# YukeWang96/GNNAdvisor_OSDI21

Measured on AMD Instinct MI355X. Metric: aggregated edges/sec, GCN sum-aggregation SpMM (SAG) hidden=64, higher is better.
Workload: dtype f32; 1 GPU; reddit-like power-law graph, random node order; num_nodes=232965, nnz=114623790, dim=64, partSize=128, num_parts=1008217, parallelism=single GPU, call=GNNA.SAG (pybind module, reference signature, fresh output), decider=auto/mi355x, column_phases=16, build_id=0.6.1+877bf822ee5a343e

## Files before the change

### gnnadvisor_osdi21_amd/build.py

```python
from __future__ import annotations

import os
import subprocess
import sys
import sysconfig

PKG = os.path.dirname(os.path.abspath(__file__))
ROOT = os.path.dirname(PKG)
CSRC = os.path.join(PKG, "csrc")
INCLUDE = os.path.join(ROOT, "include")
LIB = os.path.join(CSRC, "libgnna.so")
EXT = os.path.join(PKG, "GNNAdvisor.so")
ARCH = "gfx950"
HIPCC = os.environ.get("HIPCC", "/opt/rocm/bin/hipcc")

LIB_SOURCES = [os.path.join(CSRC, f) for f in ("gnna_agg.hip", "gnna_stream.hip", "gnna_sweep.hip", "gnna_dense.hip", "gnna_x16.hip", "gnna_reduce.hip", "gnna_stats.hip", "gnna_softagg.hip", "gnna_pool.hip", "gnna_segnorm.hip", "gnna_attnpool.hip", "gnna_topk.hip", "gnna_sddmm.hip", "gnna_edge.hip", "gnna_gat.hip", "gnna_gatv2.hip", "gnna_dotattn.hip", "gnna_typed.hip", "gnna_transpose.hip", "gnna_sample.hip", "gnna_walk.hip", "gnna_edgefeat.hip", "gnna_spatial.hip",
                                                "gnna_gemm.hip", "gnna_runtime.hip", "gnna_host.cpp", "gnna_reorder.cpp")]
PUBLIC_HEADERS = ("gnna.h", "gnna_ext.h", "gnna_gatv2.h", "gnna_dotattn.h", "gnna_gat_edge.h", "gnna_stats.h", "gnna_softagg.h",
                  "gnna_pool.h", "gnna_attnpool.h", "gnna_topk.h", "gnna_segnorm.h", "gnna_walk.h", "gnna_edgefeat.h",
                  "gnna_spatial.h")
INTERNAL_HEADERS = ("gnna_internal.h", "gnna_device.h", "gnna_launch.h", "gnna_gat_common.h", "gnna_keys.h", "gnna_segments.h",
                    "gnna_parts.h")
_PUBLIC = [os.path.join(INCLUDE, f) for f in PUBLIC_HEADERS]
LIB_DEPS = LIB_SOURCES + [os.path.join(CSRC, f) for f in INTERNAL_HEADERS] + _PUBLIC
EXT_SOURCES = [os.path.join(CSRC, "gnna_torch.cpp")]
EXT_DEPS = EXT_SOURCES + _PUBLIC


def source_hash() -> str:
    import hashlib
    h = hashlib.sha256()
    for path in sorted(set(LIB_DEPS + EXT_DEPS)):
        h.update(os.path.relpath(path, ROOT).encode() + b"\0")
        with open(path, "rb") as f:
            h.update(f.read())
        h.update(b"\0")
    return h.hexdigest()[:16]
# ... 83 lines not shown
```

### gnnadvisor_osdi21_amd/csrc/gnna_agg.hip

```cpp
#include <hip/hip_runtime.h>

#include <algorithm>
#include <cmath>
#include <cstdint>
#include <cstdio>

#include "gnna.h"
#include "gnna_device.h"
#include "gnna_internal.h"

namespace gnna {
namespace {


__global__ void __launch_bounds__(kBlock)
prologue_kernel(float *__restrict__ Y, size_t n_floats, int D, int ldy, const int32_t *__restrict__ p2n,
                const int32_t *__restrict__ pp, int64_t P, int32_t *flag, int32_t seq, int validate, int zero_fill,
                const int32_t *__restrict__ chk_ids, int64_t chk_n, const unsigned long long *__restrict__ chk_sum,
                int32_t *stale_flag, uint32_t *__restrict__ clear_words, int n_clear)
{
    if (blockIdx.x == 0 && (int)threadIdx.x < n_clear) clear_words[threadIdx.x] = 0u;
    const unsigned fill_blocks = chk_ids ? gridDim.x - 1 : gridDim.x;
    if (blockIdx.x >= fill_blocks) {
        if (threadIdx.x < kWave) {
            const unsigned long long then = chk_sum[0], distrusted = chk_sum[4];
            const unsigned long long now = graph_checksum(chk_ids, chk_n, pp, P, (int)threadIdx.x);
            if (threadIdx.x == 0 && (now != then || distrusted != 0ull)) *stale_flag = seq;
        }
        return;
    }
    const size_t tid = (size_t)blockIdx.x * blockDim.x + threadIdx.x;
    const size_t nthreads = (size_t)fill_blocks * blockDim.x;
    typedef float f32x4 __attribute__((ext_vector_type(4)));
    if (!zero_fill) {
    } else if (ldy != D) {
        if ((D & 3) == 0 && (ldy & 3) == 0 && (reinterpret_cast<uintptr_t>(Y) & 15) == 0) {
            const size_t n4 = n_floats >> 2;
            const unsigned d4 = (unsigned)D >> 2, ld4 = (unsigned)ldy >> 2;
            const f32x4 z = (f32x4)(0.f);
            for (size_t i = tid; i < n4; i += nthreads) {
                const size_t r = i / d4;
                reinterpret_cast<f32x4 *>(Y)[r * ld4 + (i - r * d4)] = z;
            }
        } else {
            for (size_t i = tid; i < n_floats; i += nthreads) {
                const size_t r = i / (unsigned)D;
                Y[r * (size_t)ldy + (i - r * (unsigned)D)] = 0.f;
            }
        }
    } else if ((reinterpret_cast<uintptr_t>(Y) & 15) == 0) {
        const size_t n4 = n_floats >> 2;
        f32x4 *Y4 = reinterpret_cast<f32x4 *>(Y);
        const f32x4 z = (f32x4)(0.f);
        for (size_t i = tid; i < n4; i += nthreads) Y4[i] = z;
        for (size_t i = (n4 << 2) + tid; i < n_floats; i += nthreads) Y[i] = 0.f;
    } else {
        for (size_t i = tid; i < n_floats; i += nthreads) Y[i] = 0.f;
    }
    if (validate) {
        bool bad = false;
        for (int64_t g = (int64_t)tid; g < P; g += (int64_t)nthreads) {
            if (pp[g + 1] < pp[g]) bad = true;
            if (g + 1 < P && p2n[g + 1] < p2n[g]) bad = true;
        }
        if (bad) *flag = seq;
    }
}

__global__ void __launch_bounds__(kBlock)
sparse_prologue_kernel(float *__restrict__ Y, int64_t N, int D, int ldy, const int32_t *__restrict__ p2n,
                       const int32_t *__restrict__ pp, int64_t P, int G, int32_t *flag, int32_t seq, int validate,
                       unsigned long long *gaps, int64_t big_rows)
{
    const int lane = threadIdx.x & (kWave - 1);
    const int64_t wave = ((int64_t)blockIdx.x * blockDim.x + threadIdx.x) >> 6;
    const int64_t nwaves = ((int64_t)gridDim.x * blockDim.x) >> 6;
    typedef float f32x4 __attribute__((ext_vector_type(4)));
    const bool vec_ok = (D & 3) == 0 && (reinterpret_cast<uintptr_t>(Y) & 15) == 0;
    auto clear_rows = [&](int64_t lo, int64_t cnt) {
        if (gaps && cnt >= big_rows) {
            unsigned long long idx = 0;
// ... 75 lines not shown
        return;
    }
    if (!gaps) return;
    const unsigned long long n = gaps[0] < (unsigned long long)kGapEntries ? gaps[0] : (unsigned long long)kGapEntries;
    for (unsigned long long k = 0; k < n; k++) {
        float *base = Y + (size_t)gaps[2 + 2 * k] * (size_t)ldy;
        const size_t cnt = (size_t)gaps[3 + 2 * k] * (size_t)D;
        for (size_t i = tid; i < cnt; i += nthreads) *at(base, i) = 0.f;
    }
}

__global__ void __launch_bounds__(kBlock)
scale_rows_kernel(const float *__restrict__ X, int64_t ld_in, const float *__restrict__ deg, float *__restrict__ Xs,
                  int64_t rows, int D, int ld_out)
{
    const size_t tid = (size_t)blockIdx.x * blockDim.x + threadIdx.x;
    const size_t nthreads = (size_t)gridDim.x * blockDim.x;
    typedef float f32x4 __attribute__((ext_vector_type(4)));
    const bool aligned = ((reinterpret_cast<uintptr_t>(X) | reinterpret_cast<uintptr_t>(Xs)) & 15) == 0;
    if (ld_out == D && ld_in == D && (D & 3) == 0 && aligned) {
        const size_t n4 = ((size_t)rows * (size_t)D) >> 2;
        const int d4 = D >> 2;
        for (size_t i = tid; i < n4; i += nthreads) {
            const f32x4 v = __builtin_nontemporal_load(reinterpret_cast<const f32x4 *>(X) + i);
            reinterpret_cast<f32x4 *>(Xs)[i] = deg ? v * deg[i / d4] : v;
        }
    } else if ((D & 3) == 0 && (ld_out & 3) == 0 && (ld_in & 3) == 0 && aligned) {
        const size_t n4 = ((size_t)rows * (size_t)D) >> 2;
        const unsigned d4 = (unsigned)D >> 2;
        const size_t ldo4 = (size_t)ld_out >> 2, ldi4 = (size_t)ld_in >> 2;
        for (size_t i = tid; i < n4; i += nthreads) {
            const size_t r = i / d4, c4 = i - r * d4;
            const f32x4 v = __builtin_nontemporal_load(reinterpret_cast<const f32x4 *>(X) + r * ldi4 + c4);
            reinterpret_cast<f32x4 *>(Xs)[r * ldo4 + c4] = deg ? v * deg[r] : v;
        }
    } else {
        const size_t total = (size_t)rows * (size_t)D;
        for (size_t i = tid; i < total; i += nthreads) {
            const size_t r = i / (unsigned)D, cc = i - r * (unsigned)D;
            const float v = __builtin_nontemporal_load(X + r * (size_t)ld_in + cc);
            Xs[r * (size_t)ld_out + cc] = deg ? v * deg[r] : v;
        }
    }
}


static size_t gather_footprint_bytes(int64_t num_in_rows, int ldx, int dim)
{
    return (size_t)num_in_rows * (size_t)std::min(ldx, (std::max(dim, 4) * 4 + 127) / 128 * 32) * sizeof(float);
}

thread_local int t_last_phases = 1;
thread_local int t_last_launches = 1;

double avg_lines_per_row(int64_t row_bytes, int64_t stride_bytes)
{
    int64_t lines = 0;
    for (int k = 0; k < 32; k++) {
// ... 81 lines not shown
    const double edges = st.edges;
    if (t.sweep != 0 || deterministic || B < 2) return 0;
    if (dim <= 32 || dim > 64 || !sweep_supports(mode, dim, x_bytes)) return 0;
    if (num_in_rows != num_out_rows || x_bytes > ((size_t)160 << 20)) return 0;
    if (edges < 300.0 * (double)std::max<int64_t>(1, num_out_rows)) return 0;
    const double cap = (double)sweep_acc_rows(dim, 1) * 0.9 * (double)std::max(8, num_cus);
    if ((double)num_out_rows > 2.0 * cap) return 0;
    if (near_share(st, (double)num_in_rows / 16.0) > 0.30) return 0;
    if (t.column_phases >= 2) return B;
    return std::max(2, std::min(std::min(16, 2 * B), std::max(2, part_size / 4)));
}

constexpr double kDenseEdgeSeconds = 9.9e-12;
constexpr double kDenseChunkSeconds = 0.73e-6;
constexpr double kDenseTallChunkSeconds = 0.76e-6;
constexpr double kDenseSplitSeconds = 11.0e-6;
constexpr double kDenseLaunchSeconds = 7.0e-6;
constexpr double kDenseMinSaving = 25.0e-6;
constexpr double kDenseMinShare = 0.03;

int trimmed_hubs(int H, int num_cus)
{
    const int round = kDenseTileRanks * std::max(1, num_cus);
    return (H > round && H % round != 0 && H % round < round / 4) ? H / round * round : H;
}

double dense_block_saving(double hubs, double entries, int num_cus)
{
    if (hubs <= 0.0) return 0.0;
    const double He = (double)trimmed_hubs((int)hubs, num_cus);
    const double Hp = std::ceil(He / kDenseChunkRanks) * kDenseChunkRanks;
// ... 72 lines not shown
    const size_t n = rows * (size_t)D;
    for (size_t i = (size_t)blockIdx.x * blockDim.x + threadIdx.x; i < n; i += (size_t)gridDim.x * blockDim.x) {
        const size_t r = i / (unsigned)D, c = i - r * (unsigned)D;
        if (Y[r * ld + c] < 0.f) Y[r * ld + c] = 0.f;
    }
}
}

void launch_relu_rows(DeviceState *ds, hipStream_t stream, float *out, int64_t rows, int dim, int64_t ld)
{
    hipLaunchKernelGGL(relu_rows_kernel, dim3(elementwise_grid(rows * dim, ds->num_cus, 8)), dim3(kBlock), 0, stream, out,
                       (size_t)ld, (size_t)rows, dim);
}

namespace {

int launch_agg(int mode, const float *input, int64_t ld_in, int64_t num_in_rows, const int32_t *column_index,
               const float *degrees, const float *degrees_in, float epsilon, const int32_t *part_pointers,
               const int32_t *part2Node, float *out, int64_t ld_out, int64_t num_nodes, int dim, int64_t num_parts,
               int partSize, int dimWorker, int warpPerBlock, void *stream_v, unsigned flags,
               int num_windows = 1, int win_begin = 0, int win_end = 1, bool profiled = true, int hint_dim = 0);

int column_blocks(const gnna_tuning &tune, int dim, int64_t num_in_rows, int64_t est_edges)
{
    if (tune.wide_blocks == 2 || dim < 72) return 1;
    if (tune.wide_blocks == 1) return (dim + 63) / 64;
    const bool hot = est_edges >= 32 * num_in_rows;
    if (!hot || (size_t)num_in_rows * (size_t)dim * sizeof(float) > ((size_t)250000000)) return 1;
    const bool long_rows = est_edges >= 200 * num_in_rows;
    if (dim < (long_rows ? 100 : 192)) return 1;
// ... 78 lines not shown
        const int nb = column_blocks(tune, dim, num_in_rows, est);
        if (nb > 1)
            return launch_agg_blocked(nb, mode, input, ld_in, num_in_rows, column_index, degrees, degrees_in, epsilon, part_pointers,
                                      part2Node, out, ld_out, num_nodes, dim, num_parts, partSize, dimWorker, warpPerBlock, stream_v, flags);
    }
    int32_t *flag = nullptr;
    const int32_t seq = next_call_seq(ds, stream, &flag);
    const int prof_call = profiled ? profile_acquire_call(num_parts > 0) : -1;
    profile_record(prof_call, 0, stream);
    const int ldy = (int)ld_out;

    const size_t n_floats = (size_t)num_nodes * (size_t)dim;
    const unsigned long long *chk_sum = nullptr;
    int64_t chk_n = 0;
    int32_t *stale_flag = flag + kFlagSlots;
    auto run_prologue = [&](int sparse_G, uint32_t *clear_words = nullptr, int n_clear = 0) -> int {
        const int validate = (num_parts > 0 && !tune.trust_canonical) ? 1 : 0;
        const int zero_fill = (accumulate_into_out || win_begin > 0) ? 0 : 1;
        if (sparse_G > 0 && zero_fill && num_parts > 0) {
            int64_t blocks = (num_parts + kBlock - 1) / kBlock;
            blocks = std::max<int64_t>(1, std::min<int64_t>(blocks, (int64_t)ds->num_cus * 8));
            unsigned long long *gaps = ds->gap_lists + (size_t)call_block_of(ds, stream, seq) * kGapWords;
            (void)hipMemsetAsync(gaps, 0, sizeof(unsigned long long), stream);
            const int64_t big_rows = std::max<int64_t>(64, ((int64_t)1 << 20) / std::max(1, dim * 4));
            hipLaunchKernelGGL(sparse_prologue_kernel, dim3((unsigned)blocks), dim3(kBlock), 0, stream, out, num_nodes, dim, ldy,
                               part2Node, part_pointers, num_parts, sparse_G, flag, seq, validate, gaps, big_rows);
            hipLaunchKernelGGL(post_prologue_kernel, dim3((unsigned)(ds->num_cus * 8)), dim3(kBlock), 0, stream, out,
                               n_floats, dim, ldy, flag, seq, gaps);
        } else {
            size_t work = std::max(n_floats / 4, (size_t)num_parts);
            int64_t blocks = (int64_t)((work + kBlock - 1) / kBlock);
            blocks = std::max<int64_t>(1, std::min<int64_t>(blocks, (int64_t)ds->num_cus * 8));
            hipLaunchKernelGGL(prologue_kernel, dim3((unsigned)blocks + (chk_sum ? 1u : 0u)), dim3(kBlock), 0, stream, out, n_floats,
                               dim, ldy, part2Node, part_pointers, num_parts, flag, seq, validate, zero_fill,
// ... 29 lines not shown
            direct = aligned16 && avg_lines_per_row((int64_t)dim * 4, ld_in * 4) <= avg_lines_per_row((int64_t)dim * 4, (int64_t)want * 4) + 1e-9;
    }
    const int ldx = direct ? (int)ld_in : want;
    const float *X = input;
    const float *row_scale = nullptr;
    float eps = epsilon;
    const size_t x_bytes = (size_t)num_in_rows * (size_t)ldx * sizeof(float);
    const size_t foot_bytes = gather_footprint_bytes(num_in_rows, ldx, dim);
    const bool wide = x_bytes > 0xffffffffull;
    if (!direct) {
        void *xs = nullptr;
        rc = get_workspace(ds, stream, 1, x_bytes, &xs);
        if (rc != GNNA_OK) return rc;
        const int64_t r0 = std::min<int64_t>((int64_t)win_begin * window_rows, num_in_rows);
        const int64_t r1 = std::min<int64_t>((int64_t)win_end * window_rows, num_in_rows);
        const size_t s_bytes = (size_t)(r1 - r0) * (size_t)dim * sizeof(float);
        int64_t sblocks = (int64_t)((s_bytes / 16 + kBlock - 1) / kBlock);
        sblocks = std::max<int64_t>(1, std::min<int64_t>(sblocks, (int64_t)ds->num_cus * 8));
        hipLaunchKernelGGL(scale_rows_kernel, dim3((unsigned)sblocks), dim3(kBlock), 0, stream,
                           input + (size_t)r0 * (size_t)ld_in, ld_in, prescale ? degrees_in + r0 : nullptr,
                           static_cast<float *>(xs) + (size_t)r0 * ldx, r1 - r0, dim, ldx);
        hipError_t es = hipGetLastError();
        if (es != hipSuccess) return fail(GNNA_ERR_HIP, "staging launch: %s", hipGetErrorString(es));
        X = static_cast<const float *>(xs);
        if (prescale) {
            row_scale = degrees;
            eps = 1.f;
            mode = MODE_GIN;
        }
    }

    int B = 1;
    const uint8_t *cnt = nullptr;
    int S = kMaxSlices;
    int win_lo = 0, win_hi = 0;
    SlicePlan plan;
    const bool can_slice = num_parts >= 1024 && num_in_rows >= 64 && foot_bytes >= ((size_t)2 << 20);
    if (windowed) {
// ... 42 lines not shown
                                tune.ids_check_every);
            if (rc != GNNA_OK) return rc;
            if (sw_ids) count_event(CTR_PACKED_LAUNCHES);
        }
        DenseBlock db;
        const int32_t *res_ids = nullptr; const uint32_t *res_off = nullptr;
        bool dense = false;
        if (sw_ids && plan.pinned && !relu && dim >= kDenseMinDim && dim <= kDenseMaxDim && num_in_rows == num_nodes && tune.column_phases < 2 &&
            plan_dense_block(plan.handle, &db) && !db.off && db.res_plan && db.res_cnt && (auto_Bs > 0 || db.forced)) {
            rc = get_packed_ids(ds, stream, db.res_plan, Bs, kWave, false, false, &res_ids, &res_off);
            if (rc != GNNA_OK) return rc;
            dense = true;
        }
        uint32_t *sync = ds->sweep_sync + (size_t)call_block_of(ds, stream, seq) * kSweepSlotWords;
        static_assert(kXcds * 16 + 2 <= kBlock, "the prologue clears the sweep counters with one block");
        rc = run_prologue(0, sync, kXcds * 16 + 2);
        if (rc != GNNA_OK) return rc;
        SweepLaunch w;
        w.mode = mode; w.X = X; w.col = column_index; w.pp = part_pointers; w.p2n = part2Node; w.Y = out;
        w.cnt = cnt; w.row_scale = row_scale; w.flag = flag; w.seq = seq; w.trust = tune.trust_canonical ? 1 : 0; w.sync = sync;
        w.P = num_parts; w.D = dim; w.ldx = ldx; w.ldy = ldy; w.S = S; w.B = Bs;
        w.relu = relu; w.num_out_rows = num_nodes;
        w.U = std::max(tune.loads_in_flight, 8);
        w.rows_with_edges = plan.stats.valid ? (int64_t)std::min((double)num_nodes, plan.stats.groups) : num_nodes;
        if (tune.groups_per_chunk > 64) w.rounds = tune.groups_per_chunk / 64;
        w.slack = tune.sweep_slack; w.wgs_per_cu = tune.blocks_per_cu;
        w.dynamic = tune.xcd_remap != 0;
        w.plain_ok = !accumulate_into_out; w.eps = eps;
        w.ids_packed = sw_ids; w.item_off = sw_off; w.packed_stale = stale_flag;
        if (dense) { w.res_col = db.res_col; w.res_pp = db.res_pp; w.res_cnt = db.res_cnt; w.res_ids_packed = res_ids; w.res_item_off = res_off; }
        t_last_phases = Bs;
        t_last_launches = 1;
        void *hub_image = nullptr;
        if (dense) {
            rc = get_workspace(ds, stream, kSlotDenseImage, dense_image_bytes(db.H_pad), &hub_image);
            if (rc != GNNA_OK) return rc;
            rc = launch_hub_split(stream, db, X, ldx, dim, hub_image, stale_flag, seq);
            if (rc != GNNA_OK) return rc;
        }
        rc = launch_sweep(ds, w, stream);
        if (rc != GNNA_OK) return rc;
        if (dense) {
            rc = launch_hub_block(ds, stream, db, hub_image, out, ldy, dim, mode == MODE_GIN, eps, row_scale, stale_flag, seq);
            if (rc != GNNA_OK) return rc;
        }
        profile_record(prof_call, 2, stream);
        return GNNA_OK;
    }

    int G = std::min(64, tune.groups_per_chunk * B);
    if (mode == MODE_EDGE && cnt && !windowed && plan.handle && plan.pinned && (plan.stats.valid || tune.sweep == 1) &&
// ... 377 lines not shown
```

### gnnadvisor_osdi21_amd/csrc/gnna_dense.hip

```cpp
#include <hip/hip_runtime.h>

#include <algorithm>
#include <cmath>
#include <cstdint>
#include <cstdio>
#include <cstdlib>
#include <vector>

#include "gnna.h"
#include "gnna_device.h"
#include "gnna_internal.h"

namespace gnna {
namespace {

constexpr int kHubBuckets = 64;
constexpr int kHubMax = 16384;
constexpr int kHubThreads = 512;
constexpr int kHubWaves = kHubThreads / kWave;
constexpr int kHubTileM = kDenseTileRanks;
constexpr int kHubKC = kDenseChunkRanks;
static_assert(kHubTileM == 32, "a tile row of the bitmap per 32 destination ranks");
constexpr int kSplitThreads = 128;
static_assert(kHubKC % (2 * kHubTileM) == 0 && (kHubTileM * 64) % kHubThreads == 0, "whole tiles per chunk, elements per thread");
static_assert(kDenseMaxDim <= 64, "the split image holds 64 columns");

__host__ __device__ inline int hub_bucket(int64_t d)
{
    if (d <= 1) return 0;
    int k = 0;
    while ((d >> (k + 1)) != 0) k++;
    const int b = 2 * k + ((d * d >= ((int64_t)1 << (2 * k + 1))) ? 1 : 0);
    return b < kHubBuckets ? b : kHubBuckets - 1;
}

__global__ void __launch_bounds__(kBlock)
hub_degree_kernel(const int32_t *__restrict__ pp, const int32_t *__restrict__ p2n, int64_t P, int64_t N, int32_t *__restrict__ deg)
{
// ... 134 lines not shown
    int32_t seq;
    int H_pad, D, ldy;
    int scaled;
    float eps;
};

struct SplitParams {
    const float *X;
    const int32_t *r2n;
    unsigned char *img;
    const int32_t *stale;
    int32_t seq;
    int D, ldx;
};

typedef typename VecOf<4>::T HubVT;
typedef int HubIT __attribute__((ext_vector_type(4)));

constexpr int kHubFrag = 1024;
constexpr int kHubPiece = 16 * kHubFrag;
constexpr int kHubImage = 3 * kHubPiece;
static_assert(kHubKC == 128 && kHubTileM == 32 && kHubWaves == 8, "the shape hub_block_kernel is written for");

typedef __bf16 HubFrag __attribute__((ext_vector_type(8)));
typedef uint32_t HubU4 __attribute__((ext_vector_type(4)));
typedef uint32_t HubU2 __attribute__((ext_vector_type(2)));

__device__ __forceinline__ void hub_split(uint32_t x, uint32_t &hi, uint32_t &mid, uint32_t &lo)
{
    hi = x & 0xffff0000u;
    const float r = __uint_as_float(x) - __uint_as_float(hi);
    mid = __float_as_uint(r) & 0xffff0000u;
    lo = __float_as_uint(r - __uint_as_float(mid));
}

__device__ __forceinline__ uint32_t hub_pack(uint32_t first, uint32_t second) { return __builtin_amdgcn_perm(second, first, 0x07060302u); }

__device__ __forceinline__ HubFrag hub_ones(uint32_t bits)
{
    const uint32_t y = bits | (bits << 15);
    HubU4 v;
#pragma unroll
    for (int i = 0; i < 4; i++) v[i] = ((y >> (2 * i)) & 0x10001u) * 0x3f80u;
    return __builtin_bit_cast(HubFrag, v);
}

template <bool FULL>
__global__ void __launch_bounds__(kSplitThreads)
hub_split_kernel(const SplitParams p)
{
    if (*p.stale == p.seq) return;
    __shared__ __attribute__((aligned(16))) unsigned char s_img[3 * 4 * kHubFrag];
    const int t = (int)threadIdx.x;
    const int g = t >> 4, pc = t & 15;
    const int step = (int)blockIdx.x;
    const int D = p.D;
    const HubIT node = *reinterpret_cast<const HubIT *>(&p.r2n[step * 32 + 4 * g]);
    HubVT v[4];
#pragma unroll
    for (int k = 0; k < 4; k++) {
        const int nd = node[k];
        const float *src = p.X + (size_t)(nd < 0 ? 0 : nd) * (size_t)p.ldx + 4 * pc;
        HubVT x = (HubVT)(0.f);
        if (nd >= 0) {
            if constexpr (FULL) {
                if (4 * pc < D) x = *reinterpret_cast<const HubVT *>(src);
            } else {
#pragma unroll
                for (int q = 0; q < 4; q++)
                    if (4 * pc + q < D) x[q] = src[q];
            }
        }
        v[k] = x;
    }
    const int wbase = (pc >> 2) * kHubFrag + (16 * (g >> 1) + 4 * (pc & 3)) * 16 + 8 * (g & 1);
#pragma unroll
    for (int cc = 0; cc < 4; cc++) {
        uint32_t pk[3][2];
#pragma unroll
        for (int h = 0; h < 2; h++) {
            uint32_t a[3], b[3];
            hub_split(__float_as_uint(v[2 * h][cc]), a[0], a[1], a[2]);
            hub_split(__float_as_uint(v[2 * h + 1][cc]), b[0], b[1], b[2]);
#pragma unroll
            for (int i = 0; i < 3; i++) pk[i][h] = hub_pack(a[i], b[i]);
        }
#pragma unroll
        for (int i = 0; i < 3; i++) {
            HubU2 o;
            o[0] = pk[i][0];
            o[1] = pk[i][1];
            *reinterpret_cast<HubU2 *>(&s_img[wbase + i * 4 * kHubFrag + cc * 16]) = o;
        }
    }
    __syncthreads();
    unsigned char *out = p.img + (size_t)(step >> 2) * kHubImage + (size_t)(step & 3) * 4 * kHubFrag;
#pragma unroll
    for (int u = 0; u < 3 * 4 * kHubFrag / 16 / kSplitThreads; u++) {
        const int idx = u * kSplitThreads + t;
        const int i = idx >> 8, off = (idx & 255) * 16;
        *reinterpret_cast<HubU4 *>(&out[i * kHubPiece + off]) = *reinterpret_cast<const HubU4 *>(&s_img[i * 4 * kHubFrag + off]);
    }
}

template <int NT, int TM>
__global__ void __launch_bounds__(kHubThreads)
hub_block_kernel(const HubParams p)
{
    if (*p.stale == p.seq) return;
    constexpr int TR = TM / 32;
    static_assert((TM == kHubTileM || TM == 2 * kHubTileM) && (NT == 3 || NT == 4), "tile shapes");
    __shared__ __attribute__((aligned(16))) float s_part[4 * TM * 64];
    const int tid = (int)threadIdx.x;
    const int lane = tid & (kWave - 1);
    const int wib = __builtin_amdgcn_readfirstlane(tid >> 6);
    const int chunks = p.H_pad / kHubKC;
    const int steps = p.H_pad >> 5;
// ... 294 lines not shown
```

### gnnadvisor_osdi21_amd/csrc/gnna_launch.h

```cpp
#ifndef GNNA_LAUNCH_H_
#define GNNA_LAUNCH_H_

#include <algorithm>
#include <cstdint>
#include <type_traits>

namespace gnna {

constexpr int kWave = 64;
constexpr int kBlock = 256;
constexpr int kWavesPerBlock = kBlock / kWave;
constexpr int kXcds = 8;

struct ChunkGrid {
    int G;
    int64_t blocks;
};
inline ChunkGrid chunk_grid(int64_t num_parts, int partSize, int num_cus)
{
    int G = std::max(1, std::min(kWave, 2048 / std::max(1, partSize)));
    while (G > 1 && (num_parts + G - 1) / G < (int64_t)num_cus * 16) G >>= 1;
    const int64_t chunks = (num_parts + G - 1) / G;
    return {G, (chunks + kWavesPerBlock - 1) / kWavesPerBlock};
}
// ... 34 lines not shown
void dispatch_layout(AttnLayout layout, F &&f)
{
    dispatch_lpr(layout.log_lph, [&](auto H) {
        dispatch_lpr(layout.log_lpr, [&](auto L) {
            if constexpr (decltype(L)::value >= decltype(H)::value) f(H, L);
        });
    });
}

inline unsigned elementwise_grid(int64_t items, int num_cus, int blocks_per_cu)
{
    const int64_t blocks = (items + kBlock - 1) / kBlock;
    return (unsigned)std::max<int64_t>(1, std::min<int64_t>(blocks, (int64_t)num_cus * blocks_per_cu));
}

inline int pow2_at_least(int64_t x)
{
    int p = 1;
    while (p < x) p <<= 1;
    return p;
}

inline bool bad_ld(int64_t ld, int64_t width) { return ld < width || ld >= ((int64_t)1 << 29); }
inline bool bad_ld_of(const void *ptr, int64_t ld, int64_t width) { return ptr ? bad_ld(ld, width) : ld >= ((int64_t)1 << 29); }

}

#endif
```

Baseline: 92.25 billion edges/s.

## Fuse staging, zero-fill, checksum and hub split into one pre-pass kernel

Merges the row-staging (degree prescale) kernel, the output zero-fill/validation prologue, the packed-id checksum check and the dense hub split into one multi-role pre-pass launch. Block roles are assigned by a grid partition that can interleave stage and fill blocks, so independent memory-bound passes share the machine and launch gaps disappear. The hub split cost constant in the dense-block cost model drops sharply, which may route more work to the dense hub path. This adds env-controlled toggles, and the single kernel carries the LDS footprint of the split role across all its blocks.

New measurement: 93.21 billion edges/s (median of 6 runs). 1.0% higher.

```diff
diff --git a/gnnadvisor_osdi21_amd/build.py b/gnnadvisor_osdi21_amd/build.py
--- a/gnnadvisor_osdi21_amd/build.py
+++ b/gnnadvisor_osdi21_amd/build.py
@@ -20,7 +20,7 @@
                   "gnna_pool.h", "gnna_attnpool.h", "gnna_topk.h", "gnna_segnorm.h", "gnna_walk.h", "gnna_edgefeat.h",
                   "gnna_spatial.h")
 INTERNAL_HEADERS = ("gnna_internal.h", "gnna_device.h", "gnna_launch.h", "gnna_gat_common.h", "gnna_keys.h", "gnna_segments.h",
-                    "gnna_parts.h")
+                    "gnna_parts.h", "gnna_prepass.h")
 _PUBLIC = [os.path.join(INCLUDE, f) for f in PUBLIC_HEADERS]
 LIB_DEPS = LIB_SOURCES + [os.path.join(CSRC, f) for f in INTERNAL_HEADERS] + _PUBLIC
 EXT_SOURCES = [os.path.join(CSRC, "gnna_torch.cpp")]
diff --git a/gnnadvisor_osdi21_amd/csrc/gnna_agg.hip b/gnnadvisor_osdi21_amd/csrc/gnna_agg.hip
--- a/gnnadvisor_osdi21_amd/csrc/gnna_agg.hip
+++ b/gnnadvisor_osdi21_amd/csrc/gnna_agg.hip
@@ -4,10 +4,12 @@
 #include <cmath>
 #include <cstdint>
 #include <cstdio>
+#include <cstdlib>
 
 #include "gnna.h"
 #include "gnna_device.h"
 #include "gnna_internal.h"
+#include "gnna_prepass.h"
 
 namespace gnna {
 namespace {
@@ -19,52 +21,13 @@
                 const int32_t *__restrict__ chk_ids, int64_t chk_n, const unsigned long long *__restrict__ chk_sum,
                 int32_t *stale_flag, uint32_t *__restrict__ clear_words, int n_clear)
 {
-    if (blockIdx.x == 0 && (int)threadIdx.x < n_clear) clear_words[threadIdx.x] = 0u;
     const unsigned fill_blocks = chk_ids ? gridDim.x - 1 : gridDim.x;
     if (blockIdx.x >= fill_blocks) {
-        if (threadIdx.x < kWave) {
-            const unsigned long long then = chk_sum[0], distrusted = chk_sum[4];
-            const unsigned long long now = graph_checksum(chk_ids, chk_n, pp, P, (int)threadIdx.x);
-            if (threadIdx.x == 0 && (now != then || distrusted != 0ull)) *stale_flag = seq;
-        }
+        check_packed_ids(chk_ids, chk_n, pp, P, chk_sum, stale_flag, seq);
         return;
     }
-    const size_t tid = (size_t)blockIdx.x * blockDim.x + threadIdx.x;
-    const size_t nthreads = (size_t)fill_blocks * blockDim.x;
-    typedef float f32x4 __attribute__((ext_vector_type(4)));
-    if (!zero_fill) {
-    } else if (ldy != D) {
-        if ((D & 3) == 0 && (ldy & 3) == 0 && (reinterpret_cast<uintptr_t>(Y) & 15) == 0) {
-            const size_t n4 = n_floats >> 2;
-            const unsigned d4 = (unsigned)D >> 2, ld4 = (unsigned)ldy >> 2;
-            const f32x4 z = (f32x4)(0.f);
-            for (size_t i = tid; i < n4; i += nthreads) {
-                const size_t r = i / d4;
-                reinterpret_cast<f32x4 *>(Y)[r * ld4 + (i - r * d4)] = z;
-            }
-        } else {
-            for (size_t i = tid; i < n_floats; i += nthreads) {
-                const size_t r = i / (unsigned)D;
-                Y[r * (size_t)ldy + (i - r * (unsigned)D)] = 0.f;
-            }
-        }
-    } else if ((reinterpret_cast<uintptr_t>(Y) & 15) == 0) {
-        const size_t n4 = n_floats >> 2;
-        f32x4 *Y4 = reinterpret_cast<f32x4 *>(Y);
-        const f32x4 z = (f32x4)(0.f);
-        for (size_t i = tid; i < n4; i += nthreads) Y4[i] = z;
-        for (size_t i = (n4 << 2) + tid; i < n_floats; i += nthreads) Y[i] = 0.f;
-    } else {
-        for (size_t i = tid; i < n_floats; i += nthreads) Y[i] = 0.f;
-    }
-    if (validate) {
-        bool bad = false;
-        for (int64_t g = (int64_t)tid; g < P; g += (int64_t)nthreads) {
-            if (pp[g + 1] < pp[g]) bad = true;
-            if (g + 1 < P && p2n[g + 1] < p2n[g]) bad = true;
-        }
-        if (bad) *flag = seq;
-    }
+    fill_and_validate(Y, n_floats, D, ldy, p2n, pp, P, flag, seq, validate, zero_fill, clear_words, n_clear, blockIdx.x, fill_blocks,
+                      blockDim.x);
 }
 
 __global__ void __launch_bounds__(kBlock)
@@ -170,34 +133,40 @@
 scale_rows_kernel(const float *__restrict__ X, int64_t ld_in, const float *__restrict__ deg, float *__restrict__ Xs,
                   int64_t rows, int D, int ld_out)
 {
-    const size_t tid = (size_t)blockIdx.x * blockDim.x + threadIdx.x;
-    const size_t nthreads = (size_t)gridDim.x * blockDim.x;
-    typedef float f32x4 __attribute__((ext_vector_type(4)));
-    const bool aligned = ((reinterpret_cast<uintptr_t>(X) | reinterpret_cast<uintptr_t>(Xs)) & 15) == 0;
-    if (ld_out == D && ld_in == D && (D & 3) == 0 && aligned) {
-        const size_t n4 = ((size_t)rows * (size_t)D) >> 2;
-        const int d4 = D >> 2;
-        for (size_t i = tid; i < n4; i += nthreads) {
-            const f32x4 v = __builtin_nontemporal_load(reinterpret_cast<const f32x4 *>(X) + i);
-            reinterpret_cast<f32x4 *>(Xs)[i] = deg ? v * deg[i / d4] : v;
-        }
-    } else if ((D & 3) == 0 && (ld_out & 3) == 0 && (ld_in & 3) == 0 && aligned) {
-        const size_t n4 = ((size_t)rows * (size_t)D) >> 2;
-        const unsigned d4 = (unsigned)D >> 2;
-        const size_t ldo4 = (size_t)ld_out >> 2, ldi4 = (size_t)ld_in >> 2;
-        for (size_t i = tid; i < n4; i += nthreads) {
-            const size_t r = i / d4, c4 = i - r * d4;
-            const f32x4 v = __builtin_nontemporal_load(reinterpret_cast<const f32x4 *>(X) + r * ldi4 + c4);
-            reinterpret_cast<f32x4 *>(Xs)[r * ldo4 + c4] = deg ? v * deg[r] : v;
-        }
-    } else {
-        const size_t total = (size_t)rows * (size_t)D;
-        for (size_t i = tid; i < total; i += nthreads) {
-            const size_t r = i / (unsigned)D, cc = i - r * (unsigned)D;
-            const float v = __builtin_nontemporal_load(X + r * (size_t)ld_in + cc);
-            Xs[r * (size_t)ld_out + cc] = deg ? v * deg[r] : v;
-        }
-    }
+    stage_rows(X, ld_in, deg, Xs, rows, D, ld_out, blockIdx.x, gridDim.x, blockDim.x);
+}
+
+struct PrepassStage { const float *X; int64_t ld_in; const float *deg; float *Xs; int64_t rows; int D; int ld_out; };
+struct PrepassFill {
+    float *Y; size_t n_floats; int D, ldy; const int32_t *p2n; const int32_t *pp; int64_t P; int32_t *flag; int32_t seq;
+    int validate, zero_fill; uint32_t *clear_words; int n_clear;
+};
+struct PrepassCheck { const int32_t *ids; int64_t n; const unsigned long long *sum; int32_t *stale_flag; };
+struct PrepassSplit { const float *X; const float *deg; const int32_t *r2n; unsigned char *img; int ldx, full; };
+
+template <bool SPLIT>
+__global__ void __launch_bounds__(kBlock)
+prepass_kernel(const PrepassGrid grid, const PrepassStage st, const PrepassFill fl, const PrepassCheck ck, const PrepassSplit sp)
+{
+    const PrepassRole r = prepass_role_of(grid, blockIdx.x);
+    if constexpr (SPLIT) {
+        __shared__ __attribute__((aligned(16))) unsigned char s_img[kSplitLdsBytes];
+        if (r.role == PREPASS_SPLIT) {
+            const int t = (int)threadIdx.x;
+            if (t < kSplitThreads) {
+                if (sp.full) split_step_to_lds<true>(sp.X, sp.ldx, sp.deg, sp.r2n, fl.D, s_img, (int)r.index, t);
+                else split_step_to_lds<false>(sp.X, sp.ldx, sp.deg, sp.r2n, fl.D, s_img, (int)r.index, t);
+            }
+            __syncthreads();
+            if (t < kSplitThreads) split_step_from_lds(sp.img, s_img, (int)r.index, t);
+            return;
+        }
+    }
+    if (r.role == PREPASS_STAGE) stage_rows(st.X, st.ld_in, st.deg, st.Xs, st.rows, st.D, st.ld_out, r.index, r.count, blockDim.x);
+    else if (r.role == PREPASS_FILL)
+        fill_and_validate(fl.Y, fl.n_floats, fl.D, fl.ldy, fl.p2n, fl.pp, fl.P, fl.flag, fl.seq, fl.validate, fl.zero_fill, fl.clear_words,
+                          fl.n_clear, r.index, r.count, blockDim.x);
+    else if (r.role == PREPASS_CHECK) check_packed_ids(ck.ids, ck.n, fl.pp, fl.P, ck.sum, ck.stale_flag, fl.seq);
 }
 
 
@@ -309,7 +278,7 @@
 constexpr double kDenseEdgeSeconds = 9.9e-12;
 constexpr double kDenseChunkSeconds = 0.73e-6;
 constexpr double kDenseTallChunkSeconds = 0.76e-6;
-constexpr double kDenseSplitSeconds = 11.0e-6;
+constexpr double kDenseSplitSeconds = 0.7e-6;
 constexpr double kDenseLaunchSeconds = 7.0e-6;
 constexpr double kDenseMinSaving = 25.0e-6;
 constexpr double kDenseMinShare = 0.03;
@@ -412,6 +381,49 @@
 }
 
 namespace {
+
+bool prepass_enabled()
+{
+    const char *s = std::getenv("GNNA_PREPASS");
+    return !(s && *s && std::atoi(s) == 0);
+}
+
+int launch_prepass(DeviceState *ds, hipStream_t stream, const PrepassStage *stage, float *out, size_t n_floats, int dim, int ldy,
+                   const int32_t *part2Node, const int32_t *part_pointers, int64_t num_parts, int32_t *flag, int32_t seq, int validate,
+                   int zero_fill, uint32_t *clear_words, int n_clear, const int32_t *chk_ids, int64_t chk_n,
+                   const unsigned long long *chk_sum, int32_t *stale_flag, const DenseBlock *split_db, const float *input, int ld_in,
+                   const float *split_deg, void *split_image)
+{
+    PrepassStage st{};
+    if (stage) st = *stage;
+    PrepassFill fl;
+    fl.Y = out; fl.n_floats = n_floats; fl.D = dim; fl.ldy = ldy; fl.p2n = part2Node; fl.pp = part_pointers; fl.P = num_parts;
+    fl.flag = flag; fl.seq = seq; fl.validate = validate; fl.zero_fill = zero_fill; fl.clear_words = clear_words; fl.n_clear = n_clear;
+    PrepassCheck ck;
+    ck.ids = chk_ids; ck.n = chk_n; ck.sum = chk_sum; ck.stale_flag = stale_flag;
+    PrepassSplit sp{};
+    if (split_db) {
+        if (dim < kDenseMinDim || dim > kDenseMaxDim) return fail(GNNA_ERR_INVALID_ARGUMENT, "hub block: width %d", dim);
+        sp.X = input; sp.deg = split_deg; sp.r2n = split_db->r2n; sp.img = static_cast<unsigned char *>(split_image); sp.ldx = ld_in;
+        sp.full = (dim % 4 == 0 && ld_in % 4 == 0 && (reinterpret_cast<uintptr_t>(input) & 15) == 0) ? 1 : 0;
+    }
+    const char *order = std::getenv("GNNA_PREPASS_ORDER");
+    const bool interleave = !(order && *order && std::atoi(order) == 0);
+    const uint64_t stage_items = stage ? (uint64_t)stage->rows * (uint64_t)dim * sizeof(float) / 16 : 0;
+    const PrepassGrid grid = prepass_grid(stage ? std::max<uint64_t>(1, stage_items) : 0,
+                                          std::max<uint64_t>(1, std::max<uint64_t>(n_floats / 4, (uint64_t)num_parts)), chk_ids != nullptr,
+                                          split_db ? (unsigned)(split_db->H_pad / 32) : 0u, ds->num_cus, interleave);
+    if (split_db) hipLaunchKernelGGL((prepass_kernel<true>), dim3(grid.total), dim3(kBlock), 0, stream, grid, st, fl, ck, sp);
+    else hipLaunchKernelGGL((prepass_kernel<false>), dim3(grid.total), dim3(kBlock), 0, stream, grid, st, fl, ck, sp);
+    hipError_t e = hipGetLastError();
+    if (e != hipSuccess) return fail(GNNA_ERR_HIP, "pre-pass launch: %s", hipGetErrorString(e));
+    const char *log = std::getenv("GNNA_PREPASS_LOG");
+    if (log && *log && *log != '0')
+        std::fprintf(stderr, "gnna prepass: stage %u, fill %u (zero-fill %d, validate %d), check %u, split %u blocks, %s\n",
+                     grid.count[PREPASS_STAGE], grid.count[PREPASS_FILL], zero_fill, validate, grid.count[PREPASS_CHECK],
+                     grid.count[PREPASS_SPLIT], interleave ? "stage and fill alternate" : "stage ahead of fill");
+    return GNNA_OK;
+}
 
 int launch_agg(int mode, const float *input, int64_t ld_in, int64_t num_in_rows, const int32_t *column_index,
                const float *degrees, const float *degrees_in, float epsilon, const int32_t *part_pointers,
@@ -520,10 +532,36 @@
     const unsigned long long *chk_sum = nullptr;
     int64_t chk_n = 0;
     int32_t *stale_flag = flag + kFlagSlots;
-    auto run_prologue = [&](int sparse_G, uint32_t *clear_words = nullptr, int n_clear = 0) -> int {
+    PrepassStage stage{};
+    bool need_stage = false, split_done = false;
+    auto run_staging = [&]() -> int {
+        const size_t s_bytes = (size_t)stage.rows * (size_t)dim * sizeof(float);
+        hipLaunchKernelGGL(scale_rows_kernel, dim3(std::max(1u, prepass_pass_blocks(s_bytes / 16, ds->num_cus))), dim3(kBlock), 0, stream,
+                           stage.X, stage.ld_in, stage.deg, stage.Xs, stage.rows, stage.D, stage.ld_out);
+        hipError_t es = hipGetLastError();
+        if (es != hipSuccess) return fail(GNNA_ERR_HIP, "staging launch: %s", hipGetErrorString(es));
+        return GNNA_OK;
+    };
+    auto run_prologue = [&](int sparse_G, uint32_t *clear_words = nullptr, int n_clear = 0, const DenseBlock *split_db = nullptr,
+                            void *split_image = nullptr) -> int {
         const int validate = (num_parts > 0 && !tune.trust_canonical) ? 1 : 0;
         const int zero_fill = (accumulate_into_out || win_begin > 0) ? 0 : 1;
-        if (sparse_G > 0 && zero_fill && num_parts > 0) {
+        const bool sparse_path = sparse_G > 0 && zero_fill && num_parts > 0;
+        if (!sparse_path && num_parts > 0 && num_windows == 1 && tune.deterministic != 1 && (need_stage || split_db) && prepass_enabled()) {
+            const int rc_pre = launch_prepass(ds, stream, need_stage ? &stage : nullptr, out, n_floats, dim, ldy, part2Node, part_pointers,
+                                              num_parts, flag, seq, validate, zero_fill, clear_words, n_clear,
+                                              chk_sum ? column_index : nullptr, chk_n, chk_sum, stale_flag, split_db, input, (int)ld_in,
+                                              stage.deg, split_image);
+            if (rc_pre != GNNA_OK) return rc_pre;
+            split_done = split_db != nullptr;
+            profile_record(prof_call, 1, stream);
+            return GNNA_OK;
+        }
+        if (need_stage) {
+            const int rc_stage = run_staging();
+            if (rc_stage != GNNA_OK) return rc_stage;
+        }
+        if (sparse_path) {
             int64_t blocks = (num_parts + kBlock - 1) / kBlock;
             blocks = std::max<int64_t>(1, std::min<int64_t>(blocks, (int64_t)ds->num_cus * 8));
             unsigned long long *gaps = ds->gap_lists + (size_t)call_block_of(ds, stream, seq) * kGapWords;
@@ -583,14 +621,9 @@
         if (rc != GNNA_OK) return rc;
         const int64_t r0 = std::min<int64_t>((int64_t)win_begin * window_rows, num_in_rows);
         const int64_t r1 = std::min<int64_t>((int64_t)win_end * window_rows, num_in_rows);
-        const size_t s_bytes = (size_t)(r1 - r0) * (size_t)dim * sizeof(float);
-        int64_t sblocks = (int64_t)((s_bytes / 16 + kBlock - 1) / kBlock);
-        sblocks = std::max<int64_t>(1, std::min<int64_t>(sblocks, (int64_t)ds->num_cus * 8));
-        hipLaunchKernelGGL(scale_rows_kernel, dim3((unsigned)sblocks), dim3(kBlock), 0, stream,
-                           input + (size_t)r0 * (size_t)ld_in, ld_in, prescale ? degrees_in + r0 : nullptr,
-                           static_cast<float *>(xs) + (size_t)r0 * ldx, r1 - r0, dim, ldx);
-        hipError_t es = hipGetLastError();
-        if (es != hipSuccess) return fail(GNNA_ERR_HIP, "staging launch: %s", hipGetErrorString(es));
+        stage.X = input + (size_t)r0 * (size_t)ld_in; stage.ld_in = ld_in; stage.deg = prescale ? degrees_in + r0 : nullptr;
+        stage.Xs = static_cast<float *>(xs) + (size_t)r0 * ldx; stage.rows = r1 - r0; stage.D = dim; stage.ld_out = ldx;
+        need_stage = true;
         X = static_cast<const float *>(xs);
         if (prescale) {
             row_scale = degrees;
@@ -663,7 +696,12 @@
         }
         uint32_t *sync = ds->sweep_sync + (size_t)call_block_of(ds, stream, seq) * kSweepSlotWords;
         static_assert(kXcds * 16 + 2 <= kBlock, "the prologue clears the sweep counters with one block");
-        rc = run_prologue(0, sync, kXcds * 16 + 2);
+        void *hub_image = nullptr;
+        if (dense) {
+            rc = get_workspace(ds, stream, kSlotDenseImage, dense_image_bytes(db.H_pad), &hub_image);
+            if (rc != GNNA_OK) return rc;
+        }
+        rc = run_prologue(0, sync, kXcds * 16 + 2, dense ? &db : nullptr, hub_image);
         if (rc != GNNA_OK) return rc;
         SweepLaunch w;
         w.mode = mode; w.X = X; w.col = column_index; w.pp = part_pointers; w.p2n = part2Node; w.Y = out;
@@ -680,10 +718,7 @@
         if (dense) { w.res_col = db.res_col; w.res_pp = db.res_pp; w.res_cnt = db.res_cnt; w.res_ids_packed = res_ids; w.res_item_off = res_off; }
         t_last_phases = Bs;
         t_last_launches = 1;
-        void *hub_image = nullptr;
-        if (dense) {
-            rc = get_workspace(ds, stream, kSlotDenseImage, dense_image_bytes(db.H_pad), &hub_image);
-            if (rc != GNNA_OK) return rc;
+        if (dense && !split_done) {
             rc = launch_hub_split(stream, db, X, ldx, dim, hub_image, stale_flag, seq);
             if (rc != GNNA_OK) return rc;
         }
diff --git a/gnnadvisor_osdi21_amd/csrc/gnna_dense.hip b/gnnadvisor_osdi21_amd/csrc/gnna_dense.hip
--- a/gnnadvisor_osdi21_amd/csrc/gnna_dense.hip
+++ b/gnnadvisor_osdi21_amd/csrc/gnna_dense.hip
@@ -10,6 +10,7 @@
 #include "gnna.h"
 #include "gnna_device.h"
 #include "gnna_internal.h"
+#include "gnna_prepass.h"
 
 namespace gnna {
 namespace {
@@ -21,7 +22,6 @@
 constexpr int kHubTileM = kDenseTileRanks;
 constexpr int kHubKC = kDenseChunkRanks;
 static_assert(kHubTileM == 32, "a tile row of the bitmap per 32 destination ranks");
-constexpr int kSplitThreads = 128;
 static_assert(kHubKC % (2 * kHubTileM) == 0 && (kHubTileM * 64) % kHubThreads == 0, "whole tiles per chunk, elements per thread");
 static_assert(kDenseMaxDim <= 64, "the split image holds 64 columns");
 
@@ -186,27 +186,8 @@
     int D, ldx;
 };
 
-typedef typename VecOf<4>::T HubVT;
-typedef int HubIT __attribute__((ext_vector_type(4)));
-
-constexpr int kHubFrag = 1024;
-constexpr int kHubPiece = 16 * kHubFrag;
-constexpr int kHubImage = 3 * kHubPiece;
+typedef __bf16 HubFrag __attribute__((ext_vector_type(8)));
 static_assert(kHubKC == 128 && kHubTileM == 32 && kHubWaves == 8, "the shape hub_block_kernel is written for");
-
-typedef __bf16 HubFrag __attribute__((ext_vector_type(8)));
-typedef uint32_t HubU4 __attribute__((ext_vector_type(4)));
-typedef uint32_t HubU2 __attribute__((ext_vector_type(2)));
-
-__device__ __forceinline__ void hub_split(uint32_t x, uint32_t &hi, uint32_t &mid, uint32_t &lo)
-{
-    hi = x & 0xffff0000u;
-    const float r = __uint_as_float(x) - __uint_as_float(hi);
-    mid = __float_as_uint(r) & 0xffff0000u;
-    lo = __float_as_uint(r - __uint_as_float(mid));
-}
-
-__device__ __forceinline__ uint32_t hub_pack(uint32_t first, uint32_t second) { return __builtin_amdgcn_perm(second, first, 0x07060302u); }
 
 __device__ __forceinline__ HubFrag hub_ones(uint32_t bits)
 {
@@ -222,57 +203,12 @@
 hub_split_kernel(const SplitParams p)
 {
     if (*p.stale == p.seq) return;
-    __shared__ __attribute__((aligned(16))) unsigned char s_img[3 * 4 * kHubFrag];
+    __shared__ __attribute__((aligned(16))) unsigned char s_img[kSplitLdsBytes];
     const int t = (int)threadIdx.x;
-    const int g = t >> 4, pc = t & 15;
     const int step = (int)blockIdx.x;
-    const int D = p.D;
-    const HubIT node = *reinterpret_cast<const HubIT *>(&p.r2n[step * 32 + 4 * g]);
-    HubVT v[4];
-#pragma unroll
-    for (int k = 0; k < 4; k++) {
-        const int nd = node[k];
-        const float *src = p.X + (size_t)(nd < 0 ? 0 : nd) * (size_t)p.ldx + 4 * pc;
-        HubVT x = (HubVT)(0.f);
-        if (nd >= 0) {
-            if constexpr (FULL) {
-                if (4 * pc < D) x = *reinterpret_cast<const HubVT *>(src);
-            } else {
-#pragma unroll
-                for (int q = 0; q < 4; q++)
-                    if (4 * pc + q < D) x[q] = src[q];
-            }
-        }
-        v[k] = x;
-    }
-    const int wbase = (pc >> 2) * kHubFrag + (16 * (g >> 1) + 4 * (pc & 3)) * 16 + 8 * (g & 1);
-#pragma unroll
-    for (int cc = 0; cc < 4; cc++) {
-        uint32_t pk[3][2];
-#pragma unroll
-        for (int h = 0; h < 2; h++) {
-            uint32_t a[3], b[3];
-            hub_split(__float_as_uint(v[2 * h][cc]), a[0], a[1], a[2]);
-            hub_split(__float_as_uint(v[2 * h + 1][cc]), b[0], b[1], b[2]);
-#pragma unroll
-            for (int i = 0; i < 3; i++) pk[i][h] = hub_pack(a[i], b[i]);
-        }
-#pragma unroll
-        for (int i = 0; i < 3; i++) {
-            HubU2 o;
-            o[0] = pk[i][0];
-            o[1] = pk[i][1];
-            *reinterpret_cast<HubU2 *>(&s_img[wbase + i * 4 * kHubFrag + cc * 16]) = o;
-        }
-    }
+    split_step_to_lds<FULL>(p.X, p.ldx, nullptr, p.r2n, p.D, s_img, step, t);
     __syncthreads();
-    unsigned char *out = p.img + (size_t)(step >> 2) * kHubImage + (size_t)(step & 3) * 4 * kHubFrag;
-#pragma unroll
-    for (int u = 0; u < 3 * 4 * kHubFrag / 16 / kSplitThreads; u++) {
-        const int idx = u * kSplitThreads + t;
-        const int i = idx >> 8, off = (idx & 255) * 16;
-        *reinterpret_cast<HubU4 *>(&out[i * kHubPiece + off]) = *reinterpret_cast<const HubU4 *>(&s_img[i * 4 * kHubFrag + off]);
-    }
+    split_step_from_lds(p.img, s_img, step, t);
 }
 
 template <int NT, int TM>
diff --git a/gnnadvisor_osdi21_amd/csrc/gnna_launch.h b/gnnadvisor_osdi21_amd/csrc/gnna_launch.h
--- a/gnnadvisor_osdi21_amd/csrc/gnna_launch.h
+++ b/gnnadvisor_osdi21_amd/csrc/gnna_launch.h
@@ -72,6 +72,57 @@
     return (unsigned)std::max<int64_t>(1, std::min<int64_t>(blocks, (int64_t)num_cus * blocks_per_cu));
 }
 
+#if defined(__HIPCC__)
+#define GNNA_HOST_DEVICE __host__ __device__
+#else
+#define GNNA_HOST_DEVICE
+#endif
+enum { PREPASS_STAGE = 0, PREPASS_FILL = 1, PREPASS_CHECK = 2, PREPASS_SPLIT = 3, PREPASS_ROLES = 4 };
+struct PrepassGrid {
+    unsigned count[PREPASS_ROLES];
+    unsigned check_begin;
+    unsigned pass_begin;
+    unsigned pairs;
+    unsigned total;
+};
+struct PrepassRole {
+    int role;
+    unsigned index, count;
+};
+inline unsigned prepass_pass_blocks(uint64_t items, int num_cus)
+{
+    if (items == 0) return 0u;
+    const uint64_t blocks = items / (uint64_t)kBlock + (items % (uint64_t)kBlock != 0 ? 1 : 0);
+    return (unsigned)std::max<uint64_t>(1, std::min<uint64_t>(blocks, (uint64_t)std::max(1, num_cus) * 8));
+}
+inline PrepassGrid prepass_grid(uint64_t stage_items, uint64_t fill_items, bool check, unsigned split_steps, int num_cus, bool interleave)
+{
+    PrepassGrid g;
+    g.count[PREPASS_STAGE] = prepass_pass_blocks(stage_items, num_cus);
+    g.count[PREPASS_FILL] = prepass_pass_blocks(fill_items, num_cus);
+    g.count[PREPASS_CHECK] = check ? 1u : 0u;
+    g.count[PREPASS_SPLIT] = split_steps;
+    g.check_begin = g.count[PREPASS_SPLIT];
+    g.pass_begin = g.check_begin + g.count[PREPASS_CHECK];
+    g.pairs = interleave ? std::min(g.count[PREPASS_STAGE], g.count[PREPASS_FILL]) : 0u;
+    g.total = g.pass_begin + g.count[PREPASS_STAGE] + g.count[PREPASS_FILL];
+    return g;
+}
+GNNA_HOST_DEVICE inline PrepassRole prepass_role_of(const PrepassGrid &g, unsigned block)
+{
+    if (block < g.check_begin) return {PREPASS_SPLIT, block, g.count[PREPASS_SPLIT]};
+    if (block < g.pass_begin) return {PREPASS_CHECK, block - g.check_begin, g.count[PREPASS_CHECK]};
+    unsigned j = block - g.pass_begin;
+    if (j < 2u * g.pairs) {
+        const int role = (j & 1u) ? PREPASS_FILL : PREPASS_STAGE;
+        return {role, j >> 1, g.count[role]};
+    }
+    j -= 2u * g.pairs;
+    const unsigned stage_left = g.count[PREPASS_STAGE] - g.pairs;
+    if (j < stage_left) return {PREPASS_STAGE, g.pairs + j, g.count[PREPASS_STAGE]};
+    return {PREPASS_FILL, g.pairs + (j - stage_left), g.count[PREPASS_FILL]};
+}
+
 inline int pow2_at_least(int64_t x)
 {
     int p = 1;
diff --git a/gnnadvisor_osdi21_amd/csrc/gnna_prepass.h b/gnnadvisor_osdi21_amd/csrc/gnna_prepass.h
--- /dev/null
+++ b/gnnadvisor_osdi21_amd/csrc/gnna_prepass.h
@@ -0,0 +1,187 @@
+#ifndef GNNA_PREPASS_H_
+#define GNNA_PREPASS_H_
+
+#include <hip/hip_runtime.h>
+
+#include <cstdint>
+
+#include "gnna_device.h"
+
+namespace gnna {
+
+__device__ __forceinline__ void stage_rows(const float *__restrict__ X, int64_t ld_in, const float *__restrict__ deg,
+                                           float *__restrict__ Xs, int64_t rows, int D, int ld_out, unsigned block, unsigned blocks,
+                                           unsigned threads)
+{
+    const size_t tid = (size_t)block * threads + threadIdx.x;
+    const size_t nthreads = (size_t)blocks * threads;
+    typedef float f32x4 __attribute__((ext_vector_type(4)));
+    const bool aligned = ((reinterpret_cast<uintptr_t>(X) | reinterpret_cast<uintptr_t>(Xs)) & 15) == 0;
+    if (ld_out == D && ld_in == D && (D & 3) == 0 && aligned) {
+        const size_t n4 = ((size_t)rows * (size_t)D) >> 2;
+        const int d4 = D >> 2;
+        for (size_t i = tid; i < n4; i += nthreads) {
+            const f32x4 v = __builtin_nontemporal_load(reinterpret_cast<const f32x4 *>(X) + i);
+            reinterpret_cast<f32x4 *>(Xs)[i] = deg ? v * deg[i / d4] : v;
+        }
+    } else if ((D & 3) == 0 && (ld_out & 3) == 0 && (ld_in & 3) == 0 && aligned) {
+        const size_t n4 = ((size_t)rows * (size_t)D) >> 2;
+        const unsigned d4 = (unsigned)D >> 2;
+        const size_t ldo4 = (size_t)ld_out >> 2, ldi4 = (size_t)ld_in >> 2;
+        for (size_t i = tid; i < n4; i += nthreads) {
+            const size_t r = i / d4, c4 = i - r * d4;
+            const f32x4 v = __builtin_nontemporal_load(reinterpret_cast<const f32x4 *>(X) + r * ldi4 + c4);
+            reinterpret_cast<f32x4 *>(Xs)[r * ldo4 + c4] = deg ? v * deg[r] : v;
+        }
+    } else {
+        const size_t total = (size_t)rows * (size_t)D;
+        for (size_t i = tid; i < total; i += nthreads) {
+            const size_t r = i / (unsigned)D, cc = i - r * (unsigned)D;
+            const float v = __builtin_nontemporal_load(X + r * (size_t)ld_in + cc);
+            Xs[r * (size_t)ld_out + cc] = deg ? v * deg[r] : v;
+        }
+    }
+}
+
+__device__ __forceinline__ void check_packed_ids(const int32_t *__restrict__ chk_ids, int64_t chk_n, const int32_t *__restrict__ pp,
+                                                 int64_t P, const unsigned long long *__restrict__ chk_sum, int32_t *stale_flag,
+                                                 int32_t seq)
+{
+    if (threadIdx.x < kWave) {
+        const unsigned long long then = chk_sum[0], distrusted = chk_sum[4];
+        const unsigned long long now = graph_checksum(chk_ids, chk_n, pp, P, (int)threadIdx.x);
+        if (threadIdx.x == 0 && (now != then || distrusted != 0ull)) *stale_flag = seq;
+    }
+}
+
+__device__ __forceinline__ void fill_and_validate(float *__restrict__ Y, size_t n_floats, int D, int ldy,
+                                                  const int32_t *__restrict__ p2n, const int32_t *__restrict__ pp, int64_t P,
+                                                  int32_t *flag, int32_t seq, int validate, int zero_fill,
+                                                  uint32_t *__restrict__ clear_words, int n_clear, unsigned block, unsigned blocks,
+                                                  unsigned threads)
+{
+    if (block == 0 && (int)threadIdx.x < n_clear) clear_words[threadIdx.x] = 0u;
+    const size_t tid = (size_t)block * threads + threadIdx.x;
+    const size_t nthreads = (size_t)blocks * threads;
+    typedef float f32x4 __attribute__((ext_vector_type(4)));
+    if (!zero_fill) {
+    } else if (ldy != D) {
+        if ((D & 3) == 0 && (ldy & 3) == 0 && (reinterpret_cast<uintptr_t>(Y) & 15) == 0) {
+            const size_t n4 = n_floats >> 2;
+            const unsigned d4 = (unsigned)D >> 2, ld4 = (unsigned)ldy >> 2;
+            const f32x4 z = (f32x4)(0.f);
+            for (size_t i = tid; i < n4; i += nthreads) {
+                const size_t r = i / d4;
+                reinterpret_cast<f32x4 *>(Y)[r * ld4 + (i - r * d4)] = z;
+            }
+        } else {
+            for (size_t i = tid; i < n_floats; i += nthreads) {
+                const size_t r = i / (unsigned)D;
+                Y[r * (size_t)ldy + (i - r * (unsigned)D)] = 0.f;
+            }
+        }
+    } else if ((reinterpret_cast<uintptr_t>(Y) & 15) == 0) {
+        const size_t n4 = n_floats >> 2;
+        f32x4 *Y4 = reinterpret_cast<f32x4 *>(Y);
+        const f32x4 z = (f32x4)(0.f);
+        for (size_t i = tid; i < n4; i += nthreads) Y4[i] = z;
+        for (size_t i = (n4 << 2) + tid; i < n_floats; i += nthreads) Y[i] = 0.f;
+    } else {
+        for (size_t i = tid; i < n_floats; i += nthreads) Y[i] = 0.f;
+    }
+    if (validate) {
+        bool bad = false;
+        for (int64_t g = (int64_t)tid; g < P; g += (int64_t)nthreads) {
+            if (pp[g + 1] < pp[g]) bad = true;
+            if (g + 1 < P && p2n[g + 1] < p2n[g]) bad = true;
+        }
+        if (bad) *flag = seq;
+    }
+}
+
+typedef typename VecOf<4>::T HubVT;
+typedef int HubIT __attribute__((ext_vector_type(4)));
+typedef uint32_t HubU4 __attribute__((ext_vector_type(4)));
+typedef uint32_t HubU2 __attribute__((ext_vector_type(2)));
+
+constexpr int kHubFrag = 1024;
+constexpr int kHubPiece = 16 * kHubFrag;
+constexpr int kHubImage = 3 * kHubPiece;
+constexpr int kSplitThreads = 128;
+constexpr int kSplitLdsBytes = 3 * 4 * kHubFrag;
+
+__device__ __forceinline__ void hub_split(uint32_t x, uint32_t &hi, uint32_t &mid, uint32_t &lo)
+{
+    hi = x & 0xffff0000u;
+    const float r = __uint_as_float(x) - __uint_as_float(hi);
+    mid = __float_as_uint(r) & 0xffff0000u;
+    lo = __float_as_uint(r - __uint_as_float(mid));
+}
+
+__device__ __forceinline__ uint32_t hub_pack(uint32_t first, uint32_t second) { return __builtin_amdgcn_perm(second, first, 0x07060302u); }
+
+template <bool FULL>
+__device__ __forceinline__ void split_step_to_lds(const float *__restrict__ X, int ldx, const float *__restrict__ deg,
+                                                  const int32_t *__restrict__ r2n, int D, unsigned char *s_img, int step, int t)
+{
+    const int g = t >> 4, pc = t & 15;
+    const HubIT node = *reinterpret_cast<const HubIT *>(&r2n[step * 32 + 4 * g]);
+    HubVT v[4];
+#pragma unroll
+    for (int k = 0; k < 4; k++) {
+        const int nd = node[k];
+        const float *src = X + (size_t)(nd < 0 ? 0 : nd) * (size_t)ldx + 4 * pc;
+        HubVT x = (HubVT)(0.f);
+        if (nd >= 0) {
+            if constexpr (FULL) {
+                if (4 * pc < D) x = *reinterpret_cast<const HubVT *>(src);
+            } else {
+#pragma unroll
+                for (int q = 0; q < 4; q++)
+                    if (4 * pc + q < D) x[q] = src[q];
+            }
+            if (deg) {
+                const float f = deg[nd];
+#pragma unroll
+                for (int q = 0; q < 4; q++)
+                    if (4 * pc + q < D) x[q] = x[q] * f;
+            }
+        }
+        v[k] = x;
+    }
+    const int wbase = (pc >> 2) * kHubFrag + (16 * (g >> 1) + 4 * (pc & 3)) * 16 + 8 * (g & 1);
+#pragma unroll
+    for (int cc = 0; cc < 4; cc++) {
+        uint32_t pk[3][2];
+#pragma unroll
+        for (int h = 0; h < 2; h++) {
+            uint32_t a[3], b[3];
+            hub_split(__float_as_uint(v[2 * h][cc]), a[0], a[1], a[2]);
+            hub_split(__float_as_uint(v[2 * h + 1][cc]), b[0], b[1], b[2]);
+#pragma unroll
+            for (int i = 0; i < 3; i++) pk[i][h] = hub_pack(a[i], b[i]);
+        }
+#pragma unroll
+        for (int i = 0; i < 3; i++) {
+            HubU2 o;
+            o[0] = pk[i][0];
+            o[1] = pk[i][1];
+            *reinterpret_cast<HubU2 *>(&s_img[wbase + i * 4 * kHubFrag + cc * 16]) = o;
+        }
+    }
+}
+
+__device__ __forceinline__ void split_step_from_lds(unsigned char *__restrict__ img, const unsigned char *s_img, int step, int t)
+{
+    unsigned char *out = img + (size_t)(step >> 2) * kHubImage + (size_t)(step & 3) * 4 * kHubFrag;
+#pragma unroll
+    for (int u = 0; u < kSplitLdsBytes / 16 / kSplitThreads; u++) {
+        const int idx = u * kSplitThreads + t;
+        const int i = idx >> 8, off = (idx & 255) * 16;
+        *reinterpret_cast<HubU4 *>(&out[i * kHubPiece + off]) = *reinterpret_cast<const HubU4 *>(&s_img[i * 4 * kHubFrag + off]);
+    }
+}
+
+}
+
+#endif
```
